# fdeguire03/InteriorPoint-GPU

Measured on AMD Instinct MI355X. Metric: Newton iters/sec, dense QP n=8192, 1/2/4/8 GPUs; achieved % fp64 roofline, higher is better.
Workload: dtype f64

## Files before the change

### interiorpoint-gpu_amd/csrc/ipm_mfma.h

```cpp
#pragma once
#include <algorithm>
#include <map>
#include <mutex>
#include <queue>
#include <tuple>
#include <type_traits>
#include <vector>

#include "ipm_common.h"

namespace ipm {

#ifdef IPM_TILE_STAMPS
__device__ unsigned long long ipm_tile_stamps[4096 * 8];
#define IPM_TSTAMP(k) do { if (threadIdx.x == 0 && blockIdx.x < 4096) ipm_tile_stamps[blockIdx.x * 8 + (k)] = __builtin_amdgcn_s_memtime(); } while (0)
#define IPM_TSTAMPR(k) do { if (threadIdx.x == 0 && blockIdx.x < 4096) ipm_tile_stamps[blockIdx.x * 8 + (k)] = __builtin_amdgcn_s_memrealtime(); } while (0)
#else
#define IPM_TSTAMP(k) do {} while (0)
#define IPM_TSTAMPR(k) do {} while (0)
#endif

struct GemmArgs {
  int64_t ni = 0, nj = 0, K = 0;
  const double* X = nullptr;
  int64_t ldx = 0;
  const double* Y = nullptr;
  int64_t ldy = 0;
  const double* w = nullptr;
  double* C = nullptr;
  int64_t ldc = 0;
  double alpha = 1.0, beta = 0.0;
  const double* P = nullptr;
  int64_t ldp = 0;
  double tP = 0.0;
  const double* dvec = nullptr;
  const int* info = nullptr;
  int tri = 0;
  int sub = 0;
  int xcd_remap = 1;
  int rowmajor = 0;
  int64_t tiles_i = 0, tiles_j = 0, nblk = 0;
  int accum = 0;
};

#define IPM_KARGS(T, name, param) \
  (void)param;                    \
  const T& name = *(const T*)__builtin_amdgcn_kernarg_segment_ptr()

__device__ __forceinline__ double ld_sc1(const double* p) {
  return __longlong_as_double((long long)__hip_atomic_load(
      reinterpret_cast<unsigned long long*>(const_cast<double*>(p)), __ATOMIC_RELAXED, __HIP_MEMORY_SCOPE_AGENT));
}
__device__ __forceinline__ void st_sc1(double* p, double v) {
  __hip_atomic_store(reinterpret_cast<unsigned long long*>(p), (unsigned long long)__double_as_longlong(v),
                     __ATOMIC_RELAXED, __HIP_MEMORY_SCOPE_AGENT);
}

static __device__ unsigned long long ipm_spin_ticks[2] = {100000000ull, 100000000ull};
__device__ __forceinline__ void spin_fail(int* info, unsigned* failw) {
  if (info) atomicCAS(info, 0, POTRF_INFO_SPIN);
  __threadfence();
  if (failw) atomicCAS(failw, 0u, 0xFFFFFFF0u);
}
template <int SLEEP, int WHICH = 0, class Done>
__device__ __forceinline__ bool spin_until(int* info, unsigned* failw, Done done) {
  if (done()) return true;
  unsigned long long t0 = 0;
  for (unsigned it = 0;; ++it) {
    __builtin_amdgcn_s_sleep(SLEEP);
    if (done()) return true;
    if ((it & 15u) != 0u) continue;
    const unsigned long long now = __builtin_amdgcn_s_memrealtime();
    if (it == 0) {
      t0 = now;
      continue;
    }
    if (failw && __hip_atomic_load(failw, __ATOMIC_RELAXED, __HIP_MEMORY_SCOPE_AGENT) != 0u) return false;
    if (now - t0 > ipm_spin_ticks[WHICH]) {
      spin_fail(info, failw);
      return false;
    }
  }
}

#ifndef IPM_STILE_XRING
#define IPM_STILE_XRING 3
#endif

template <int BM_, int WJ = 2>
struct MfCfg {
  static constexpr int BM = BM_, BK = 16, NT = 128 * WJ;
  static constexpr int LD = BM + 16;
  static constexpr int PT = BK * BM / NT;
  static constexpr int TPR = BM / PT;
  static constexpr int TWI = BM / 32;
  static constexpr int TWJ = BM / (16 * WJ);
};

template <int BM_, int WJ = 2>
struct alignas(16) MfSmem {
  alignas(16) double sX[2][MfCfg<BM_, WJ>::BK * MfCfg<BM_, WJ>::LD];
  alignas(16) double sY[2][MfCfg<BM_, WJ>::BK * MfCfg<BM_, WJ>::LD];
};

template <int BM_, bool WEIGHT, bool VEC, int WJ = 2, bool SC1OUT = false, bool SPLITADD = false, int LOOP = 0,
          int LAZYC = 0, bool CST = false>
__device__ __forceinline__ void mfma_tile(const GemmArgs& a, int64_t Lw, MfSmem<BM_, WJ>& sm, int SPLIT = 0,
                                          double* part = nullptr, unsigned* pflag = nullptr, int64_t kb = -1,
                                          int64_t ke = -1, int* sinfo = nullptr, unsigned* failw = nullptr) {
  using M = MfCfg<BM_, WJ>;
  constexpr int BM = M::BM, BK = M::BK, LD = M::LD, PT = M::PT, TPR = M::TPR, TWI = M::TWI, TWJ = M::TWJ;
  IPM_TSTAMP(0);
  IPM_TSTAMPR(6);
#ifdef IPM_TILE_STAMPS
  if (threadIdx.x == 0 && blockIdx.x < 4096)
    ipm_tile_stamps[blockIdx.x * 8 + 5] = ((unsigned long long)__builtin_amdgcn_s_getreg((31 << 11) | 20) << 32) |
                                          __builtin_amdgcn_s_getreg((31 << 11) | 4);
#endif
  auto& sX = sm.sX;
  auto& sY = sm.sY;
  int64_t bi, bj;
  {
    int64_t L = Lw;
    const int64_t q = a.nblk >> 3;
    if (a.xcd_remap && !a.rowmajor && L < (q << 3)) L = (L & 7) * q + (L >> 3);
    if (a.rowmajor) {
      bi = L / a.tiles_j;
      bj = L % a.tiles_j;
    } else if (a.tri) {
      int64_t b = (int64_t)((sqrt(8.0 * (double)L + 1.0) - 1.0) * 0.5);
      while ((b + 1) * (b + 2) / 2 <= L) ++b;
      while (b * (b + 1) / 2 > L) --b;
      bi = b;
      bj = L - b * (b + 1) / 2;
    } else {
      bi = L % a.tiles_i;
      bj = L / a.tiles_i;
    }
  }
  const int64_t I0 = bi * BM, J0 = bj * BM;
  const bool full = (I0 + BM <= a.ni) && (J0 + BM <= a.nj);
  const int tid = threadIdx.x, lane = tid & 63, wv = tid >> 6;
  const int wi = wv & 1, wj = wv >> 1;
  const int sr = tid / TPR, sc = (tid % TPR) * PT;
  const bool kpiece = SPLITADD && kb >= 0;
  const int64_t kbeg = SPLIT == 1 ? (kpiece ? kb : a.K / 2) : 0;
  const double* xp = a.X + (sr + kbeg) * a.ldx + I0 + sc;
  const double* yp = a.Y + (sr + kbeg) * a.ldy + J0 + sc;
  const int64_t xstep = BK * a.ldx, ystep = BK * a.ldy;
  int kt32 = (int)a.K;
  if (SPLIT == 1) kt32 = kpiece ? (int)(ke - kb) : kt32 - kt32 / 2;
  if (SPLIT == 2) kt32 = kt32 / 2;
  const int64_t Kt = kt32;
  const int64_t nslab = (Kt + BK - 1) / BK;
  const bool cinit = a.sub || a.accum || (a.beta == 1.0 && a.alpha == -1.0 && !a.P && !a.dvec);
  const double xsg = (cinit && !a.accum) ? -1.0 : 1.0;
  double rx[PT], ry[PT];
  auto gload = [&](int64_t s) {
    const int64_t k = s * BK + sr;
    const double* xs = xp + s * xstep;
    const double* ys = yp + s * ystep;
    if (full && (s + 1) * BK <= Kt) {
      const double wk = WEIGHT ? a.w[kbeg + k] : 1.0;
      if (VEC) {
#pragma unroll
        for (int q = 0; q < PT / 2; ++q) {
          const double2 u = reinterpret_cast<const double2*>(xs)[q];
          const double2 v = reinterpret_cast<const double2*>(ys)[q];
          rx[2 * q] = (WEIGHT ? u.x * wk : u.x) * xsg;
          rx[2 * q + 1] = (WEIGHT ? u.y * wk : u.y) * xsg;
          ry[2 * q] = v.x;
          ry[2 * q + 1] = v.y;
        }
      } else {
#pragma unroll
        for (int q = 0; q < PT; ++q) {
          rx[q] = (WEIGHT ? xs[q] * wk : xs[q]) * xsg;
          ry[q] = ys[q];
        }
      }
    } else {
      const bool kin = k < Kt;
      const double wk = (WEIGHT && kin) ? a.w[kbeg + k] : 1.0;
#pragma unroll
      for (int q = 0; q < PT; ++q) {
        const bool xi = kin && (I0 + sc + q < a.ni), yj = kin && (J0 + sc + q < a.nj);
        rx[q] = xi ? (WEIGHT ? xs[q] * wk : xs[q]) * xsg : 0.0;
        ry[q] = yj ? ys[q] : 0.0;
      }
    }
  };
  auto sstore = [&](int buf) {
#pragma unroll
    for (int q = 0; q < PT; ++q) {
      sX[buf][sr * LD + sc + q] = rx[q];
      sY[buf][sr * LD + sc + q] = ry[q];
    }
  };
  const int fr = lane & 15, fk = lane >> 4;
  dbl4 acc[TWJ][TWI];
#pragma unroll
  for (int u = 0; u < TWJ; ++u)
#pragma unroll
    for (int v = 0; v < TWI; ++v) acc[u][v] = dbl4{0.0, 0.0, 0.0, 0.0};
  static_assert(!LAZYC || ((LOOP == 1 || LOOP == 2) && !WEIGHT), "lazy C: a fast loop, no weight");
  static_assert(!CST || (LOOP == 1 && !LAZYC && BM_ == 128 && WJ == 2), "staged C: 128-tile fast loop");
  constexpr int CLD = 144;
  double* sCst = &sm.sX[0][0];
  static_assert(!CST || 4 * BK * LD >= 64 * CLD, "staging fits the slab buffers");
  if (CST && cinit && SPLIT == 0) {
#pragma unroll
    for (int h = 0; h < 2; ++h) {
#pragma unroll
      for (int q = 0; q < 16; ++q) {
        const int e = tid + 256 * q, col = e >> 6, rp = e & 63;
        const double2 v = *reinterpret_cast<const double2*>(a.C + (J0 + 64 * h + col) * a.ldc + I0 + 2 * rp);
        *reinterpret_cast<double2*>(&sCst[col * CLD + 2 * rp]) = v;
      }
      __syncthreads();
      if (wj == h) {
#pragma unroll
        for (int tj = 0; tj < TWJ; ++tj)
#pragma unroll
          for (int ti = 0; ti < TWI; ++ti)
#pragma unroll
            for (int r = 0; r < 4; ++r)
              acc[tj][ti][r] = sCst[(tj * 16 + fk + 4 * r) * CLD + wi * (BM / 2) + ti * 16 + fr];
      }
      __syncthreads();
    }
  } else if (cinit && SPLIT != 1 && !LAZYC) {
#pragma unroll
    for (int tj = 0; tj < TWJ; ++tj)
#pragma unroll
      for (int ti = 0; ti < TWI; ++ti) {
        const int64_t i = I0 + wi * (BM / 2) + ti * 16 + fr;
#pragma unroll
        for (int r = 0; r < 4; ++r) {
          const int64_t j = J0 + wj * (BM / WJ) + tj * 16 + fk + 4 * r;
          acc[tj][ti][r] = (i < a.ni && j < a.nj) ? (SC1OUT ? ld_sc1(&a.C[j * a.ldc + i]) : a.C[j * a.ldc + i]) : 0.0;
        }
      }
  }
  static_assert(LOOP == 0 || (BM_ == 128 && VEC && WJ == 2), "fast loop: 128-tiles, vector loads");
  if constexpr (LAZYC) {
    auto cload = [&](int q) {
      const int tj = q / TWI, ti = q % TWI;
      const int64_t i = I0 + wi * (BM / 2) + ti * 16 + fr;
      const int64_t j0 = J0 + wj * (BM / WJ) + tj * 16 + fk;
      dbl4 v;
#pragma unroll
      for (int r = 0; r < 4; ++r) v[r] = a.C[(j0 + 4 * r) * a.ldc + i];
      return v;
    };
    constexpr int NS = 16, R = LAZYC > 0 ? LAZYC : 1, NSL = NS * R;
    static_assert(TWJ * TWI == NS, "one accumulator block per R slabs");
    dbl4 cq[NS];
    if constexpr (LOOP == 2) {
      double fy[PT];
      auto fload = [&](int64_t s) {
        const double2* ys = reinterpret_cast<const double2*>(yp + s * ystep);
#pragma unroll
        for (int q = 0; q < PT / 2; ++q) {
          const double2 v = ys[q];
          fy[2 * q] = v.x;
          fy[2 * q + 1] = v.y;
        }
      };
      auto fstore = [&](int buf) {
#pragma unroll
        for (int q = 0; q < PT; ++q) sY[buf][sr * LD + sc + q] = fy[q];
      };
      const double* xq = a.X + (kbeg + fk) * a.ldx + I0 + wi * (BM / 2) + fr;
      constexpr int XRING = IPM_STILE_XRING, G = NSL * (BK / 4);
      double xr[XRING][TWI];
// ... 214 lines not shown
#pragma unroll
      for (int t = 0; t < TWJ; ++t) yr[kk][t] = q[t * 16];
      if (WEIGHT) wk[kk] = wq[s * BK + kk * 4];
    };
#pragma unroll
    for (int kk = 0; kk < BK / 4; ++kk) load(0, kk);
    for (int64_t s = 0; s < nslab; ++s) {
      const int64_t sn = std::min<int64_t>(s + 1, nslab - 1);
#pragma unroll
      for (int kk = 0; kk < BK / 4; ++kk) {
        double av[TWJ], bv[TWI];
#pragma unroll
        for (int t = 0; t < TWJ; ++t) av[t] = yr[kk][t];
#pragma unroll
        for (int t = 0; t < TWI; ++t) bv[t] = (WEIGHT ? xr[kk][t] * wk[kk] : xr[kk][t]) * xsg;
        load(sn, kk);
#pragma unroll
        for (int tj = 0; tj < TWJ; ++tj)
#pragma unroll
          for (int ti = 0; ti < TWI; ++ti)
            acc[tj][ti] = __builtin_amdgcn_mfma_f64_16x16x4f64(av[tj], bv[ti], acc[tj][ti], 0, 0, 0);
      }
    }
  } else {
    if (nslab > 0) {
      gload(0);
      sstore(0);
      if (nslab > 1) gload(1);
    }
    __syncthreads();
    for (int64_t s = 0; s < nslab; ++s) {
      const int buf = (int)(s & 1);
      const double* bx = sX[buf];
      const double* by = sY[buf];
  #pragma unroll
      for (int kk = 0; kk < BK / 4; ++kk) {
        double av[TWJ], bv[TWI];
  #pragma unroll
        for (int t = 0; t < TWJ; ++t) av[t] = by[(kk * 4 + fk) * LD + wj * (BM / WJ) + t * 16 + fr];
  #pragma unroll
        for (int t = 0; t < TWI; ++t) bv[t] = bx[(kk * 4 + fk) * LD + wi * (BM / 2) + t * 16 + fr];
  #pragma unroll
        for (int tj = 0; tj < TWJ; ++tj)
  #pragma unroll
          for (int ti = 0; ti < TWI; ++ti)
            acc[tj][ti] = __builtin_amdgcn_mfma_f64_16x16x4f64(av[tj], bv[ti], acc[tj][ti], 0, 0, 0);
      }
      if (s + 1 < nslab) {
        sstore(buf ^ 1);
        if (s + 2 < nslab) gload(s + 2);
      }
      __syncthreads();
    }
  }
  if (SPLIT == 2) {
    if (tid == 0)
      spin_until<2>(sinfo, failw, [&] { return __hip_atomic_load(pflag, __ATOMIC_RELAXED, __HIP_MEMORY_SCOPE_AGENT) != 0u; });
    __syncthreads();
  }
  if (CST && cinit && SPLIT == 0) {
    const bool diag = a.tri && I0 == J0;
#pragma unroll
    for (int h = 0; h < 2; ++h) {
      if (wj == h) {
#pragma unroll
        for (int tj = 0; tj < TWJ; ++tj)
#pragma unroll
          for (int ti = 0; ti < TWI; ++ti)
#pragma unroll
            for (int r = 0; r < 4; ++r)
              sCst[(tj * 16 + fk + 4 * r) * CLD + wi * (BM / 2) + ti * 16 + fr] = acc[tj][ti][r];
      }
      __syncthreads();
#pragma unroll
      for (int q = 0; q < 16; ++q) {
        const int e = tid + 256 * q, col = e >> 6, rp = e & 63;
        const double2 v = *reinterpret_cast<const double2*>(&sCst[col * CLD + 2 * rp]);
        double* cp = a.C + (J0 + 64 * h + col) * a.ldc + I0 + 2 * rp;
        const int c = 64 * h + col;
        if (!diag || 2 * rp >= c) {
          *reinterpret_cast<double2*>(cp) = v;
        } else if (2 * rp + 1 == c) {
          cp[1] = v.y;
        }
      }
      if (h == 0) __syncthreads();
    }
    return;
  }
  constexpr bool PRE = LOOP >= 2 && !LAZYC;
#pragma unroll
  for (int tj = 0; tj < TWJ; ++tj) {
    double pp[TWI][4], pc[TWI][4];
    if constexpr (PRE) {
      if (!cinit && SPLIT != 1) {
#pragma unroll
        for (int ti = 0; ti < TWI; ++ti) {
          const int64_t i = I0 + wi * (BM / 2) + ti * 16 + fr;
#pragma unroll
          for (int r = 0; r < 4; ++r) {
            const int64_t j = J0 + wj * (BM / WJ) + tj * 16 + fk + 4 * r;
            const bool ok = i < a.ni && j < a.nj && (!a.tri || i >= j);
            pp[ti][r] = (ok && a.P) ? a.P[j * a.ldp + i] : 0.0;
            pc[ti][r] = (ok && a.beta != 0.0) ? a.C[j * a.ldc + i] : 0.0;
          }
        }
      }
    }
#pragma unroll
    for (int ti = 0; ti < TWI; ++ti) {
      const int64_t i = I0 + wi * (BM / 2) + ti * 16 + fr;
#pragma unroll
      for (int r = 0; r < 4; ++r) {
        const int64_t j = J0 + wj * (BM / WJ) + tj * 16 + fk + 4 * r;
        if (SPLIT == 1) {
          st_sc1(&part[(j - J0) * BM + (i - I0)], acc[tj][ti][r]);
        } else if (i < a.ni && j < a.nj && (!a.tri || i >= j)) {
          double* cp = a.C + j * a.ldc + i;
          if (cinit) {
            double v = acc[tj][ti][r];
            if (SPLIT == 2) v += ld_sc1(&part[(j - J0) * BM + (i - I0)]);
            if (SC1OUT) st_sc1(cp, v);
            else *cp = v;
          } else {
            double av = acc[tj][ti][r];
            if (SPLITADD && SPLIT == 2) av += ld_sc1(&part[(j - J0) * BM + (i - I0)]);
            double v = a.alpha * av;
            if (a.beta != 0.0) v += a.beta * (PRE ? pc[ti][r] : *cp);
            if (a.P) v += a.tP * (PRE ? pp[ti][r] : a.P[j * a.ldp + i]);
            if (a.dvec && i == j) v += a.dvec[i];
            *cp = v;
          }
        }
      }
    }
  }
  if (SPLIT == 1) {
    asm volatile("s_waitcnt vmcnt(0)" ::: "memory");
    __syncthreads();
    if (tid == 0) __hip_atomic_store(pflag, 1u, __ATOMIC_RELAXED, __HIP_MEMORY_SCOPE_AGENT);
  }
  if (SPLIT == 2) {
    __syncthreads();
    if (tid == 0) __hip_atomic_store(pflag, 0u, __ATOMIC_RELAXED, __HIP_MEMORY_SCOPE_AGENT);
  }
#ifdef IPM_TILE_STAMPS
  IPM_TSTAMP(3);
  asm volatile("s_waitcnt vmcnt(0)" ::: "memory");
  IPM_TSTAMP(4);
  IPM_TSTAMPR(7);
#endif
}

template <int BM>
__device__ __forceinline__ bool tile_fast_ok(const GemmArgs& a, int64_t Lw) {
  int64_t L = Lw, bi, bj;
  const int64_t q = a.nblk >> 3;
  if (a.xcd_remap && !a.rowmajor && L < (q << 3)) L = (L & 7) * q + (L >> 3);
  if (a.rowmajor) {
    bi = L / a.tiles_j;
    bj = L % a.tiles_j;
  } else if (a.tri) {
    int64_t b = (int64_t)((sqrt(8.0 * (double)L + 1.0) - 1.0) * 0.5);
    while ((b + 1) * (b + 2) / 2 <= L) ++b;
    while (b * (b + 1) / 2 > L) --b;
    bi = b;
    bj = L - b * (b + 1) / 2;
  } else {
    bi = L % a.tiles_i;
    bj = L / a.tiles_i;
  }
  return (bi + 1) * BM <= a.ni && (bj + 1) * BM <= a.nj && (a.K % 16) == 0;
}

#ifndef IPM_SYRK_LOOP
#define IPM_SYRK_LOOP 2
#endif

template <int BM_, bool WEIGHT, bool VEC, int WJ = 2>
__global__ __launch_bounds__(128 * WJ, 2 / (WJ / 2)) void k_mfma_gemm(GemmArgs a) {
  if (a.info && *a.info != 0) return;
  __shared__ MfSmem<BM_, WJ> sm;
  for (int64_t Lw = blockIdx.x; Lw < a.nblk; Lw += gridDim.x) {
    if (BM_ == 128 && VEC && WJ == 2 && tile_fast_ok<BM_>(a, Lw))
      mfma_tile<BM_, WEIGHT, VEC, WJ, false, false, (BM_ == 128 && VEC && WJ == 2) ? IPM_SYRK_LOOP : 0>(a, Lw, sm);
    else
      mfma_tile<BM_, WEIGHT, VEC, WJ>(a, Lw, sm);
  }
}

template <int BM_, bool WEIGHT, bool VEC>
__global__ __launch_bounds__(256, 2) void k_mfma_gemm_split(GemmArgs a, int64_t s_full, double* sscr,
                                                            unsigned* sflag) {
  if (a.info && *a.info != 0) return;
  __shared__ MfSmem<BM_, 2> sm;
  const int64_t b = blockIdx.x;
  constexpr int FL = (BM_ == 128 && VEC) ? IPM_SYRK_LOOP : 0;
  if (b < s_full) {
    if (FL && tile_fast_ok<BM_>(a, b)) mfma_tile<BM_, WEIGHT, VEC, 2, false, true, FL>(a, b, sm);
    else mfma_tile<BM_, WEIGHT, VEC, 2, false, true>(a, b, sm);
    return;
  }
  const int64_t u = b - s_full, p = u >> 1;
  double* part = sscr + p * (int64_t)(BM_ * BM_);
  const int64_t Lw = s_full + p;
  if (FL && (a.K % 32) == 0 && tile_fast_ok<BM_>(a, Lw))
    mfma_tile<BM_, WEIGHT, VEC, 2, false, true, FL>(a, Lw, sm, (u & 1) ? 2 : 1, part, sflag + p);
  else
    mfma_tile<BM_, WEIGHT, VEC, 2, false, true>(a, Lw, sm, (u & 1) ? 2 : 1, part, sflag + p);
}

template <int BM>
__device__ __forceinline__ void tile_ij(const GemmArgs& a, int64_t Lw, int64_t& bi, int64_t& bj) {
  int64_t L = Lw;
  const int64_t q = a.nblk >> 3;
  if (a.xcd_remap && !a.rowmajor && L < (q << 3)) L = (L & 7) * q + (L >> 3);
  if (a.rowmajor) {
    bi = L / a.tiles_j;
    bj = L % a.tiles_j;
  } else if (a.tri) {
    int64_t b = (int64_t)((sqrt(8.0 * (double)L + 1.0) - 1.0) * 0.5);
    while ((b + 1) * (b + 2) / 2 <= L) ++b;
    while (b * (b + 1) / 2 > L) --b;
    bi = b;
    bj = L - b * (b + 1) / 2;
  } else {
    bi = L % a.tiles_i;
    bj = L / a.tiles_i;
  }
}

template <bool WEIGHT, bool VEC>
__global__ __launch_bounds__(256, 2) void k_mfma_gemm_streamk(GemmArgs a, int64_t s_full, int P, int64_t Kp,
                                                              int64_t npc, double* sscr, unsigned* cnt,
                                                              int pieces_last) {
  constexpr int BM = 128;
  if (a.info && *a.info != 0) return;
  __shared__ MfSmem<BM, 2> sm;
  __shared__ int slast;
  int64_t b = blockIdx.x;
  constexpr int FL = VEC ? IPM_SYRK_LOOP : 0;
  bool whole;
  if (pieces_last) {
    whole = b < s_full;
    if (!whole) b -= s_full;
  } else {
    whole = b >= npc;
  }
  if (whole) {
    const int64_t L = pieces_last ? b : b - npc;
    if (FL && tile_fast_ok<BM>(a, L)) mfma_tile<BM, WEIGHT, VEC, 2, false, true, FL>(a, L, sm);
    else mfma_tile<BM, WEIGHT, VEC, 2, false, true>(a, L, sm);
    return;
  }
  const int64_t ti = b / P, p = b - ti * P, L = s_full + ti;
  const int64_t k0 = p * Kp, k1 = std::min<int64_t>(a.K, k0 + Kp);
  double* part = sscr + b * (int64_t)(BM * BM);
  unsigned* pf = cnt + (a.nblk - s_full) + b;
  if (FL && (k0 % 16) == 0 && ((k1 - k0) % 16) == 0 && tile_fast_ok<BM>(a, L))
    mfma_tile<BM, WEIGHT, VEC, 2, false, true, FL>(a, L, sm, 1, part, pf, k0, k1);
  else
    mfma_tile<BM, WEIGHT, VEC, 2, false, true>(a, L, sm, 1, part, pf, k0, k1);
  const int tid = threadIdx.x;
  if (tid == 0)
    slast = __hip_atomic_fetch_add(&cnt[ti], 1u, __ATOMIC_RELAXED, __HIP_MEMORY_SCOPE_AGENT) == (unsigned)(P - 1);
  __syncthreads();
  if (!slast) return;
  int64_t bi, bj;
  tile_ij<BM>(a, L, bi, bj);
  const int64_t I0 = bi * BM, J0 = bj * BM;
  const bool cinit = a.sub || a.accum || (a.beta == 1.0 && a.alpha == -1.0 && !a.P && !a.dvec);
  const double* base = sscr + ti * P * (int64_t)(BM * BM);
  auto fixup = [&](auto pc) {
    constexpr int NP = decltype(pc)::value, U = NP >= 8 ? 4 : 8;
    for (int e0 = tid; e0 < BM * BM; e0 += U * 256) {
      double pv[U][NP], pp[U], cv[U];
#pragma unroll
      for (int u = 0; u < U; ++u)
#pragma unroll
        for (int q = 0; q < NP; ++q) pv[u][q] = ld_sc1(&base[q * (int64_t)(BM * BM) + e0 + 256 * u]);
      bool ok[U];
#pragma unroll
      for (int u = 0; u < U; ++u) {
        const int e = e0 + 256 * u;
        const int64_t i = I0 + (e & (BM - 1)), j = J0 + e / BM;
        ok[u] = !(i >= a.ni || j >= a.nj || (a.tri && i < j));
        pp[u] = (ok[u] && !cinit && a.P) ? a.P[j * a.ldp + i] : 0.0;
        cv[u] = (ok[u] && (cinit || a.beta != 0.0)) ? a.C[j * a.ldc + i] : 0.0;
      }
#pragma unroll
      for (int u = 0; u < U; ++u) {
        if (!ok[u]) continue;
        const int e = e0 + 256 * u;
        const int64_t i = I0 + (e & (BM - 1)), j = J0 + e / BM;
        double sum = 0.0;
#pragma unroll
        for (int q = 0; q < NP; ++q) sum += pv[u][q];
        double* cp = a.C + j * a.ldc + i;
        if (cinit) {
          *cp = cv[u] + sum;
        } else {
          double v = a.alpha * sum;
          if (a.beta != 0.0) v += a.beta * cv[u];
          if (a.P) v += a.tP * pp[u];
          if (a.dvec && i == j) v += a.dvec[i];
          *cp = v;
        }
      }
    }
  };
  if (P == 16) fixup(std::integral_constant<int, 16>{});
  else if (P == 8) fixup(std::integral_constant<int, 8>{});
  else if (P == 4) fixup(std::integral_constant<int, 4>{});
  else {
    for (int e = tid; e < BM * BM; e += 256) {
      const int il = e & (BM - 1), jl = e / BM;
      const int64_t i = I0 + il, j = J0 + jl;
      if (i >= a.ni || j >= a.nj || (a.tri && i < j)) continue;
      double pv[16];
#pragma unroll
      for (int q = 0; q < 16; ++q) pv[q] = q < P ? ld_sc1(&base[q * (int64_t)(BM * BM) + e]) : 0.0;
      double sum = 0.0;
#pragma unroll
      for (int q = 0; q < 16; ++q)
        if (q < P) sum += pv[q];
      double* cp = a.C + j * a.ldc + i;
      if (cinit) {
        *cp = *cp + sum;
      } else {
        double v = a.alpha * sum;
        if (a.beta != 0.0) v += a.beta * (*cp);
        if (a.P) v += a.tP * a.P[j * a.ldp + i];
        if (a.dvec && i == j) v += a.dvec[i];
        *cp = v;
      }
    }
  }
  IPM_TSTAMPR(7);
  if (tid == 0) __hip_atomic_store(&cnt[ti], 0u, __ATOMIC_RELAXED, __HIP_MEMORY_SCOPE_AGENT);
}

inline int streamk_mode(int64_t nt = 0, int slots = 0) {
  static const int env = [] {
    const char* e = getenv("IPM_STREAMK");
    return e ? atoi(e) : -1;
  }();
  if (env >= 0) return env;
  (void)nt;
  (void)slots;
  return 2;
}
inline int streamk_plan(int64_t nt, int slots, int64_t cap, int64_t K, int64_t& q, int64_t& Kp) {
  const int mode = streamk_mode(nt, slots);
  q = 0;
  Kp = 0;
  if (!mode || slots <= 0 || nt < slots) return 0;
  q = nt % slots;
  if (q == 0) return 0;
  const int pmax = (mode == 3 || mode == 4) ? 8 : 16;
  int P = 1;
  while (P * 2 <= pmax && q * P * 2 <= slots && q * P * 2 <= cap && K / (P * 2) >= 64) P *= 2;
  if (P < 4) return 0;
  Kp = ((K + P - 1) / P + 15) / 16 * 16;
  P = (int)((K + Kp - 1) / Kp);
  return P >= 4 ? P : 0;
}

inline int64_t gemm_split_plan(int64_t nt, int slots, int64_t cap) {
  if (nt <= 0 || slots <= 0) return 0;
  static std::mutex mu;
  static std::map<std::tuple<int64_t, int, int64_t>, int64_t> cache;
  std::lock_guard<std::mutex> lk(mu);
  const auto key = std::make_tuple(nt, slots, cap);
  auto it = cache.find(key);
  if (it != cache.end()) return it->second;
  auto mk = [&](int64_t q) {
    std::priority_queue<double, std::vector<double>, std::greater<double>> pq;
    for (int i = 0; i < slots; ++i) pq.push(0.0);
    double m = 0.0;
    auto put = [&](double d) {
      const double t = pq.top() + d;
      pq.pop();
      pq.push(t);
      m = std::max(m, t);
    };
    for (int64_t i = 0; i < nt - q; ++i) put(1.0);
    for (int64_t i = 0; i < 2 * q; ++i) put(0.55);
    return m;
  };
  double best = mk(0);
  int64_t bq = 0;
  for (int64_t q = 8; q <= std::min(nt, cap); q += 8) {
    const double m = mk(q);
    if (m < best - 0.02) {
      best = m;
      bq = q;
    }
  }
  cache[key] = bq;
  return bq;
}

template <int BM>
inline void mfma_gemm_launch_bm(hipStream_t st, GemmArgs a, bool vec) {
  const int64_t ti = (a.ni + BM - 1) / BM, tj = (a.nj + BM - 1) / BM;
  a.tiles_i = ti;
  a.nblk = a.tri ? ti * (ti + 1) / 2 : ti * tj;
  dim3 g((unsigned)a.nblk), b(256);
  if (a.w) {
    if (vec) hipLaunchKernelGGL((k_mfma_gemm<BM, true, true>), g, b, 0, st, a);
    else hipLaunchKernelGGL((k_mfma_gemm<BM, true, false>), g, b, 0, st, a);
  } else {
    if (vec) hipLaunchKernelGGL((k_mfma_gemm<BM, false, true>), g, b, 0, st, a);
    else hipLaunchKernelGGL((k_mfma_gemm<BM, false, false>), g, b, 0, st, a);
  }
}

inline void mfma_gemm_launch(hipStream_t st, GemmArgs a) {
  if (a.ni <= 0 || a.nj <= 0) return;
  const bool vec = ((a.ldx & 1) == 0) && ((a.ldy & 1) == 0) && ((((uintptr_t)a.X) & 15) == 0) &&
                   ((((uintptr_t)a.Y) & 15) == 0);
  const int64_t ti = (a.ni + 127) / 128, tj = (a.nj + 127) / 128;
  const int64_t nblk128 = a.tri ? ti * (ti + 1) / 2 : ti * tj;
  if (nblk128 >= 768) mfma_gemm_launch_bm<128>(st, a, vec);
  else mfma_gemm_launch_bm<64>(st, a, vec);
}

inline void mfma_gemm_launch_split(hipStream_t st, GemmArgs a, double* ws, int64_t cap, int slots,
                                   bool flags_zero = false) {
  if (a.ni <= 0 || a.nj <= 0) return;
  const bool vec = ((a.ldx & 1) == 0) && ((a.ldy & 1) == 0) && ((((uintptr_t)a.X) & 15) == 0) &&
                   ((((uintptr_t)a.Y) & 15) == 0);
  const int64_t ti128 = (a.ni + 127) / 128, tj128 = (a.nj + 127) / 128;
  const int64_t nblk128 = a.tri ? ti128 * (ti128 + 1) / 2 : ti128 * tj128;
  int BM = nblk128 >= 768 ? 128 : 64;
  if (BM == 64 && ws) {
    int64_t q0 = 0, K0 = 0;
    if (streamk_plan(nblk128, slots, cap, a.K, q0, K0) > 0) BM = 128;
  }
  const int64_t ti = (a.ni + BM - 1) / BM, tj = (a.nj + BM - 1) / BM;
  a.tiles_i = ti;
  a.nblk = a.tri ? ti * (ti + 1) / 2 : ti * tj;
  if (BM == 128 && ws) {
    int64_t qk = 0, Kp = 0;
    const int P = streamk_plan(a.nblk, slots, cap, a.K, qk, Kp);
    if (P > 0) {
      const int64_t s_full = a.nblk - qk, npc = qk * P;
      unsigned* cnt = reinterpret_cast<unsigned*>(ws + cap * (int64_t)(128 * 128));
      if (!flags_zero) hipMemsetAsync(cnt, 0, qk * sizeof(unsigned), st);
      dim3 g((unsigned)(npc + s_full)), blk(256);
      const int pl = (streamk_mode(a.nblk, slots) == 2 || streamk_mode(a.nblk, slots) == 4) ? 1 : 0;
      if (a.w) {
        if (vec) hipLaunchKernelGGL((k_mfma_gemm_streamk<true, true>), g, blk, 0, st, a, s_full, P, Kp, npc, ws, cnt, pl);
        else hipLaunchKernelGGL((k_mfma_gemm_streamk<true, false>), g, blk, 0, st, a, s_full, P, Kp, npc, ws, cnt, pl);
      } else {
        if (vec) hipLaunchKernelGGL((k_mfma_gemm_streamk<false, true>), g, blk, 0, st, a, s_full, P, Kp, npc, ws, cnt, pl);
        else hipLaunchKernelGGL((k_mfma_gemm_streamk<false, false>), g, blk, 0, st, a, s_full, P, Kp, npc, ws, cnt, pl);
      }
      return;
    }
  }
  const int64_t q = ws ? gemm_split_plan(a.nblk, slots, std::min<int64_t>(cap, 256)) : 0;
  if (q == 0) {
    if (BM == 128) mfma_gemm_launch_bm<128>(st, a, vec);
    else mfma_gemm_launch_bm<64>(st, a, vec);
    return;
  }
  const int64_t s_full = a.nblk - q;
  unsigned* flags = reinterpret_cast<unsigned*>(ws + cap * (int64_t)(128 * 128));
  if (!flags_zero) hipMemsetAsync(flags, 0, q * sizeof(unsigned), st);
  dim3 g((unsigned)(s_full + 2 * q)), b(256);
#define IPM_SPLIT_LAUNCH(BMv)                                                                             \
  do {                                                                                                    \
    if (a.w) {                                                                                            \
      if (vec) hipLaunchKernelGGL((k_mfma_gemm_split<BMv, true, true>), g, b, 0, st, a, s_full, ws, flags);   \
      else hipLaunchKernelGGL((k_mfma_gemm_split<BMv, true, false>), g, b, 0, st, a, s_full, ws, flags);      \
    } else {                                                                                              \
      if (vec) hipLaunchKernelGGL((k_mfma_gemm_split<BMv, false, true>), g, b, 0, st, a, s_full, ws, flags);  \
      else hipLaunchKernelGGL((k_mfma_gemm_split<BMv, false, false>), g, b, 0, st, a, s_full, ws, flags);     \
    }                                                                                                     \
  } while (0)
  if (BM == 128) IPM_SPLIT_LAUNCH(128);
  else IPM_SPLIT_LAUNCH(64);
#undef IPM_SPLIT_LAUNCH
}

}
```

Measured before the change: 124.0.

## Add diagonal-tile SYRK path computing only lower-triangle 16x16 blocks per wave

Adds a specialized kernel path for diagonal 128x128 tiles of triangular (SYRK-style) GEMMs. Each of the four waves computes exactly 9 of the 36 lower-triangle 16x16 sub-blocks, statically verified to cover the triangle, instead of the full tile. Tile ordering can now place diagonal tiles last, and a host-side load-balancing planner (diag_plan) weighs diagonal tiles at 36/64 cost when choosing between stream-K, split, or plain launches and between BM=64 and BM=128. This skips the MFMA work on upper-triangle blocks of diagonal tiles, at the cost of more template instantiations, register pressure from the unrolled per-wave schedule, and more complex scheduling heuristics.

```diff
diff --git a/interiorpoint-gpu_amd/csrc/ipm_mfma.h b/interiorpoint-gpu_amd/csrc/ipm_mfma.h
--- a/interiorpoint-gpu_amd/csrc/ipm_mfma.h
+++ b/interiorpoint-gpu_amd/csrc/ipm_mfma.h
@@ -5,6 +5,7 @@
 #include <queue>
 #include <tuple>
 #include <type_traits>
+#include <utility>
 #include <vector>
 
 #include "ipm_common.h"
@@ -42,6 +43,7 @@
   int64_t tiles_i = 0, tiles_j = 0, nblk = 0;
   int accum = 0;
 };
+constexpr int TRI_SHORT = 2, TRI_DLAST = 4;
 
 #define IPM_KARGS(T, name, param) \
   (void)param;                    \
@@ -103,8 +105,23 @@
   alignas(16) double sY[2][MfCfg<BM_, WJ>::BK * MfCfg<BM_, WJ>::LD];
 };
 
+__device__ __forceinline__ void tri_dlast_ij(const GemmArgs& a, int64_t L, int64_t& bi, int64_t& bj) {
+  const int64_t ns = a.tiles_i * (a.tiles_i - 1) / 2;
+  if (L >= ns) {
+    bi = bj = L - ns;
+    return;
+  }
+  const int64_t q = ns >> 3;
+  if (a.xcd_remap && L < (q << 3)) L = (L & 7) * q + (L >> 3);
+  int64_t b = (int64_t)((sqrt(8.0 * (double)L + 1.0) - 1.0) * 0.5);
+  while ((b + 1) * (b + 2) / 2 <= L) ++b;
+  while (b * (b + 1) / 2 > L) --b;
+  bi = b + 1;
+  bj = L - b * (b + 1) / 2;
+}
+
 template <int BM_, bool WEIGHT, bool VEC, int WJ = 2, bool SC1OUT = false, bool SPLITADD = false, int LOOP = 0,
-          int LAZYC = 0, bool CST = false>
+          int LAZYC = 0, bool CST = false, bool DLAST = false>
 __device__ __forceinline__ void mfma_tile(const GemmArgs& a, int64_t Lw, MfSmem<BM_, WJ>& sm, int SPLIT = 0,
                                           double* part = nullptr, unsigned* pflag = nullptr, int64_t kb = -1,
                                           int64_t ke = -1, int* sinfo = nullptr, unsigned* failw = nullptr) {
@@ -120,7 +137,9 @@
   auto& sX = sm.sX;
   auto& sY = sm.sY;
   int64_t bi, bj;
-  {
+  if (DLAST && (a.tri & TRI_DLAST)) {
+    tri_dlast_ij(a, Lw, bi, bj);
+  } else {
     int64_t L = Lw;
     const int64_t q = a.nblk >> 3;
     if (a.xcd_remap && !a.rowmajor && L < (q << 3)) L = (L & 7) * q + (L >> 3);
@@ -641,9 +660,13 @@
 #endif
 }
 
-template <int BM>
+template <int BM, bool DLAST = false>
 __device__ __forceinline__ bool tile_fast_ok(const GemmArgs& a, int64_t Lw) {
   int64_t L = Lw, bi, bj;
+  if (DLAST && (a.tri & TRI_DLAST)) {
+    tri_dlast_ij(a, Lw, bi, bj);
+    return (bi + 1) * BM <= a.ni && (bj + 1) * BM <= a.nj && (a.K % 16) == 0;
+  }
   const int64_t q = a.nblk >> 3;
   if (a.xcd_remap && !a.rowmajor && L < (q << 3)) L = (L & 7) * q + (L >> 3);
   if (a.rowmajor) {
@@ -662,6 +685,224 @@
   return (bi + 1) * BM <= a.ni && (bj + 1) * BM <= a.nj && (a.K % 16) == 0;
 }
 
+template <int W>
+struct DiagPart;
+template <>
+struct DiagPart<0> {
+  static constexpr int NX = 5, NY = 2;
+  static constexpr int xr[5] = {4, 5, 6, 7, 0}, yc[5] = {0, 1, 0, 0, 0};
+  static constexpr int bx[9] = {0, 0, 1, 1, 2, 2, 3, 3, 4}, by[9] = {0, 1, 0, 1, 0, 1, 0, 1, 0};
+};
+template <>
+struct DiagPart<1> {
+  static constexpr int NX = 5, NY = 3;
+  static constexpr int xr[5] = {4, 5, 6, 7, 1}, yc[5] = {2, 3, 1, 0, 0};
+  static constexpr int bx[9] = {0, 0, 1, 1, 2, 2, 3, 3, 4}, by[9] = {0, 1, 0, 1, 0, 1, 0, 1, 2};
+};
+template <>
+struct DiagPart<2> {
+  static constexpr int NX = 4, NY = 5;
+  static constexpr int xr[5] = {1, 2, 3, 4, 0}, yc[5] = {0, 1, 2, 3, 4};
+  static constexpr int bx[9] = {0, 1, 1, 1, 2, 2, 2, 2, 3}, by[9] = {0, 0, 1, 2, 0, 1, 2, 3, 4};
+};
+template <>
+struct DiagPart<3> {
+  static constexpr int NX = 3, NY = 4;
+  static constexpr int xr[5] = {5, 6, 7, 0, 0}, yc[5] = {4, 5, 6, 7, 0};
+  static constexpr int bx[9] = {0, 0, 1, 1, 1, 2, 2, 2, 2}, by[9] = {0, 1, 0, 1, 2, 0, 1, 2, 3};
+};
+template <int W>
+constexpr unsigned long long diag_part_mask() {
+  using P = DiagPart<W>;
+  unsigned long long m = 0;
+  for (int n = 0; n < 9; ++n) {
+    const int br = P::xr[P::bx[n]], bc = P::yc[P::by[n]];
+    if (P::bx[n] >= P::NX || P::by[n] >= P::NY || br < bc || ((m >> (8 * br + bc)) & 1ull)) return 0;
+    m |= 1ull << (8 * br + bc);
+  }
+  return m;
+}
+constexpr unsigned long long diag_lower_mask() {
+  unsigned long long m = 0;
+  for (int br = 0; br < 8; ++br)
+    for (int bc = 0; bc <= br; ++bc) m |= 1ull << (8 * br + bc);
+  return m;
+}
+static_assert((diag_part_mask<0>() & diag_part_mask<1>()) == 0 && (diag_part_mask<2>() & diag_part_mask<3>()) == 0 &&
+                  ((diag_part_mask<0>() | diag_part_mask<1>()) & (diag_part_mask<2>() | diag_part_mask<3>())) == 0 &&
+                  (diag_part_mask<0>() | diag_part_mask<1>() | diag_part_mask<2>() | diag_part_mask<3>()) ==
+                      diag_lower_mask(),
+              "the four waves' blocks: an exact 9 / 9 / 9 / 9 cover of the lower triangle");
+
+template <class F, int... I>
+__device__ __forceinline__ void static_for_impl(F&& f, std::integer_sequence<int, I...>) {
+  (f(std::integral_constant<int, I>{}), ...);
+}
+template <int N, class F>
+__device__ __forceinline__ void static_for(F&& f) {
+  static_for_impl(f, std::make_integer_sequence<int, N>{});
+}
+
+template <int W, bool WEIGHT>
+__device__ __forceinline__ void mfma_diag_wave(const GemmArgs& a, int64_t I0, MfSmem<128, 2>& sm) {
+  using M = MfCfg<128, 2>;
+  using P = DiagPart<W>;
+  constexpr int BK = M::BK, LD = M::LD, PT = M::PT, TPR = M::TPR, NX = P::NX, NY = P::NY, NB = 9;
+  auto& sY = sm.sY;
+  const int64_t J0 = I0;
+  const int tid = threadIdx.x, lane = tid & 63;
+  const int sr = tid / TPR, sc = (tid % TPR) * PT;
+  const int fr = lane & 15, fk = lane >> 4;
+  const double* yp = a.Y + sr * a.ldy + J0 + sc;
+  const int64_t ystep = BK * a.ldy;
+  const int64_t nslab = a.K / BK;
+  const bool cinit = a.sub || a.accum || (a.beta == 1.0 && a.alpha == -1.0 && !a.P && !a.dvec);
+  const double xsg = (cinit && !a.accum) ? -1.0 : 1.0;
+  dbl4 acc[NB];
+#pragma unroll
+  for (int n = 0; n < NB; ++n) acc[n] = dbl4{0.0, 0.0, 0.0, 0.0};
+  if (cinit) {
+    static_for<NB>([&](auto ic) {
+      constexpr int n = decltype(ic)::value, br = P::xr[P::bx[n]], bc = P::yc[P::by[n]];
+      const int64_t i = I0 + br * 16 + fr;
+#pragma unroll
+      for (int r = 0; r < 4; ++r) acc[n][r] = a.C[(J0 + bc * 16 + fk + 4 * r) * a.ldc + i];
+    });
+  }
+  double fy[PT];
+  auto fload = [&](int64_t s) {
+    const double2* ys = reinterpret_cast<const double2*>(yp + s * ystep);
+#pragma unroll
+    for (int q = 0; q < PT / 2; ++q) {
+      const double2 v = ys[q];
+      fy[2 * q] = v.x;
+      fy[2 * q + 1] = v.y;
+    }
+  };
+  auto fstore = [&](int buf) {
+#pragma unroll
+    for (int q = 0; q < PT; ++q) sY[buf][sr * LD + sc + q] = fy[q];
+  };
+  const double* xq = a.X + fk * a.ldx + I0 + fr;
+  const double* wq = WEIGHT ? a.w + fk : nullptr;
+  double xr[BK / 4][NX], wk[BK / 4];
+  auto xload = [&](int64_t s, int kk) {
+    const double* p = xq + (s * BK + kk * 4) * a.ldx;
+    static_for<NX>([&](auto tc) {
+      constexpr int t = decltype(tc)::value;
+      xr[kk][t] = p[P::xr[t] * 16];
+    });
+    if (WEIGHT) wk[kk] = wq[s * BK + kk * 4];
+  };
+  fload(0);
+  fstore(0);
+  fload(nslab > 1 ? 1 : 0);
+#pragma unroll
+  for (int kk = 0; kk < BK / 4; ++kk) xload(0, kk);
+  __syncthreads();
+  IPM_TSTAMP(1);
+  for (int64_t s = 0; s < nslab; ++s) {
+    const int buf = (int)(s & 1);
+    const double* by = sY[buf];
+    fstore(buf ^ 1);
+    fload(std::min<int64_t>(s + 2, nslab - 1));
+    const int64_t sn = std::min<int64_t>(s + 1, nslab - 1);
+    __builtin_amdgcn_sched_barrier(0);
+#pragma unroll
+    for (int kk = 0; kk < BK / 4; ++kk) {
+      double av[NY], bv[NX];
+      static_for<NY>([&](auto tc) {
+        constexpr int t = decltype(tc)::value;
+        av[t] = by[(kk * 4 + fk) * LD + P::yc[t] * 16 + fr];
+      });
+#pragma unroll
+      for (int t = 0; t < NX; ++t) bv[t] = (WEIGHT ? xr[kk][t] * wk[kk] : xr[kk][t]) * xsg;
+      xload(sn, kk);
+      static_for<NB>([&](auto ic) {
+        constexpr int n = decltype(ic)::value;
+        acc[n] = __builtin_amdgcn_mfma_f64_16x16x4f64(av[P::by[n]], bv[P::bx[n]], acc[n], 0, 0, 0);
+      });
+    }
+    __syncthreads();
+  }
+  IPM_TSTAMP(2);
+  static_for<NB / 3>([&](auto gc) {
+    constexpr int g = decltype(gc)::value;
+    double pp[3][4], pc[3][4];
+    if (!cinit) {
+      static_for<3>([&](auto uc) {
+        constexpr int u = decltype(uc)::value, n = 3 * g + u, br = P::xr[P::bx[n]], bc = P::yc[P::by[n]];
+        const int64_t i = I0 + br * 16 + fr;
+#pragma unroll
+        for (int r = 0; r < 4; ++r) {
+          const int64_t j = J0 + bc * 16 + fk + 4 * r;
+          const bool ok = br > bc || i >= j;
+          pp[u][r] = (ok && a.P) ? a.P[j * a.ldp + i] : 0.0;
+          pc[u][r] = (ok && a.beta != 0.0) ? a.C[j * a.ldc + i] : 0.0;
+        }
+      });
+    }
+    static_for<3>([&](auto uc) {
+      constexpr int u = decltype(uc)::value, n = 3 * g + u, br = P::xr[P::bx[n]], bc = P::yc[P::by[n]];
+      const int64_t i = I0 + br * 16 + fr;
+#pragma unroll
+      for (int r = 0; r < 4; ++r) {
+        const int64_t j = J0 + bc * 16 + fk + 4 * r;
+        if (br > bc || i >= j) {
+          double* cp = a.C + j * a.ldc + i;
+          if (cinit) {
+            *cp = acc[n][r];
+          } else {
+            double v = a.alpha * acc[n][r];
+            if (a.beta != 0.0) v += a.beta * pc[u][r];
+            if (a.P) v += a.tP * pp[u][r];
+            if (a.dvec && i == j) v += a.dvec[i];
+            *cp = v;
+          }
+        }
+      }
+    });
+  });
+}
+
+template <bool WEIGHT>
+__device__ __forceinline__ void mfma_tile_diag(const GemmArgs& a, int64_t I0, MfSmem<128, 2>& sm) {
+  IPM_TSTAMP(0);
+  IPM_TSTAMPR(6);
+  switch (__builtin_amdgcn_readfirstlane((int)(threadIdx.x >> 6))) {
+    case 0: mfma_diag_wave<0, WEIGHT>(a, I0, sm); break;
+    case 1: mfma_diag_wave<1, WEIGHT>(a, I0, sm); break;
+    case 2: mfma_diag_wave<2, WEIGHT>(a, I0, sm); break;
+    default: mfma_diag_wave<3, WEIGHT>(a, I0, sm); break;
+  }
+#ifdef IPM_TILE_STAMPS
+  IPM_TSTAMP(3);
+  asm volatile("s_waitcnt vmcnt(0)" ::: "memory");
+  IPM_TSTAMP(4);
+  IPM_TSTAMPR(7);
+#endif
+}
+
+template <int BM>
+__device__ __forceinline__ bool tile_diag_ok(const GemmArgs& a, int64_t Lw, int64_t& I0) {
+  if (BM != 128 || !(a.tri & TRI_SHORT)) return false;
+  int64_t bi, bj;
+  if (a.tri & TRI_DLAST) {
+    tri_dlast_ij(a, Lw, bi, bj);
+  } else {
+    int64_t L = Lw;
+    const int64_t q = a.nblk >> 3;
+    if (a.xcd_remap && L < (q << 3)) L = (L & 7) * q + (L >> 3);
+    int64_t b = (int64_t)((sqrt(8.0 * (double)L + 1.0) - 1.0) * 0.5);
+    while ((b + 1) * (b + 2) / 2 <= L) ++b;
+    while (b * (b + 1) / 2 > L) --b;
+    bi = b;
+    bj = L - b * (b + 1) / 2;
+  }
+  I0 = bi * 128;
+  return bi == bj && I0 + 128 <= a.ni && a.K >= 16 && (a.K % 16) == 0;
+}
+
 #ifndef IPM_SYRK_LOOP
 #define IPM_SYRK_LOOP 2
 #endif
@@ -678,6 +919,16 @@
   }
 }
 
+template <bool WEIGHT>
+__global__ __launch_bounds__(256, 2) void k_mfma_syrk_diag(GemmArgs a) {
+  if (a.info && *a.info != 0) return;
+  __shared__ MfSmem<128, 2> sm;
+  const int64_t Lw = blockIdx.x;
+  int64_t D0;
+  if (tile_diag_ok<128>(a, Lw, D0)) mfma_tile_diag<WEIGHT>(a, D0, sm);
+  else mfma_tile<128, WEIGHT, true, 2, false, false, IPM_SYRK_LOOP, 0, false, true>(a, Lw, sm);
+}
+
 template <int BM_, bool WEIGHT, bool VEC>
 __global__ __launch_bounds__(256, 2) void k_mfma_gemm_split(GemmArgs a, int64_t s_full, double* sscr,
                                                             unsigned* sflag) {
@@ -686,21 +937,32 @@
   const int64_t b = blockIdx.x;
   constexpr int FL = (BM_ == 128 && VEC) ? IPM_SYRK_LOOP : 0;
   if (b < s_full) {
-    if (FL && tile_fast_ok<BM_>(a, b)) mfma_tile<BM_, WEIGHT, VEC, 2, false, true, FL>(a, b, sm);
-    else mfma_tile<BM_, WEIGHT, VEC, 2, false, true>(a, b, sm);
+    if constexpr (BM_ == 128 && VEC) {
+      int64_t D0;
+      if (tile_diag_ok<BM_>(a, b, D0)) {
+        mfma_tile_diag<WEIGHT>(a, D0, sm);
+        return;
+      }
+    }
+    if (FL && tile_fast_ok<BM_, true>(a, b)) mfma_tile<BM_, WEIGHT, VEC, 2, false, true, FL, 0, false, true>(a, b, sm);
+    else mfma_tile<BM_, WEIGHT, VEC, 2, false, true, 0, 0, false, true>(a, b, sm);
     return;
   }
   const int64_t u = b - s_full, p = u >> 1;
   double* part = sscr + p * (int64_t)(BM_ * BM_);
   const int64_t Lw = s_full + p;
-  if (FL && (a.K % 32) == 0 && tile_fast_ok<BM_>(a, Lw))
-    mfma_tile<BM_, WEIGHT, VEC, 2, false, true, FL>(a, Lw, sm, (u & 1) ? 2 : 1, part, sflag + p);
+  if (FL && (a.K % 32) == 0 && tile_fast_ok<BM_, true>(a, Lw))
+    mfma_tile<BM_, WEIGHT, VEC, 2, false, true, FL, 0, false, true>(a, Lw, sm, (u & 1) ? 2 : 1, part, sflag + p);
   else
-    mfma_tile<BM_, WEIGHT, VEC, 2, false, true>(a, Lw, sm, (u & 1) ? 2 : 1, part, sflag + p);
+    mfma_tile<BM_, WEIGHT, VEC, 2, false, true, 0, 0, false, true>(a, Lw, sm, (u & 1) ? 2 : 1, part, sflag + p);
 }
 
 template <int BM>
 __device__ __forceinline__ void tile_ij(const GemmArgs& a, int64_t Lw, int64_t& bi, int64_t& bj) {
+  if (a.tri & TRI_DLAST) {
+    tri_dlast_ij(a, Lw, bi, bj);
+    return;
+  }
   int64_t L = Lw;
   const int64_t q = a.nblk >> 3;
   if (a.xcd_remap && !a.rowmajor && L < (q << 3)) L = (L & 7) * q + (L >> 3);
@@ -738,18 +1000,25 @@
   }
   if (whole) {
     const int64_t L = pieces_last ? b : b - npc;
-    if (FL && tile_fast_ok<BM>(a, L)) mfma_tile<BM, WEIGHT, VEC, 2, false, true, FL>(a, L, sm);
-    else mfma_tile<BM, WEIGHT, VEC, 2, false, true>(a, L, sm);
+    if constexpr (VEC) {
+      int64_t D0;
+      if (tile_diag_ok<BM>(a, L, D0)) {
+        mfma_tile_diag<WEIGHT>(a, D0, sm);
+        return;
+      }
+    }
+    if (FL && tile_fast_ok<BM, true>(a, L)) mfma_tile<BM, WEIGHT, VEC, 2, false, true, FL, 0, false, true>(a, L, sm);
+    else mfma_tile<BM, WEIGHT, VEC, 2, false, true, 0, 0, false, true>(a, L, sm);
     return;
   }
   const int64_t ti = b / P, p = b - ti * P, L = s_full + ti;
   const int64_t k0 = p * Kp, k1 = std::min<int64_t>(a.K, k0 + Kp);
   double* part = sscr + b * (int64_t)(BM * BM);
   unsigned* pf = cnt + (a.nblk - s_full) + b;
-  if (FL && (k0 % 16) == 0 && ((k1 - k0) % 16) == 0 && tile_fast_ok<BM>(a, L))
-    mfma_tile<BM, WEIGHT, VEC, 2, false, true, FL>(a, L, sm, 1, part, pf, k0, k1);
+  if (FL && (k0 % 16) == 0 && ((k1 - k0) % 16) == 0 && tile_fast_ok<BM, true>(a, L))
+    mfma_tile<BM, WEIGHT, VEC, 2, false, true, FL, 0, false, true>(a, L, sm, 1, part, pf, k0, k1);
   else
-    mfma_tile<BM, WEIGHT, VEC, 2, false, true>(a, L, sm, 1, part, pf, k0, k1);
+    mfma_tile<BM, WEIGHT, VEC, 2, false, true, 0, 0, false, true>(a, L, sm, 1, part, pf, k0, k1);
   const int tid = threadIdx.x;
   if (tid == 0)
     slast = __hip_atomic_fetch_add(&cnt[ti], 1u, __ATOMIC_RELAXED, __HIP_MEMORY_SCOPE_AGENT) == (unsigned)(P - 1);
@@ -829,11 +1098,15 @@
   if (tid == 0) __hip_atomic_store(&cnt[ti], 0u, __ATOMIC_RELAXED, __HIP_MEMORY_SCOPE_AGENT);
 }
 
-inline int streamk_mode(int64_t nt = 0, int slots = 0) {
+inline int streamk_env() {
   static const int env = [] {
     const char* e = getenv("IPM_STREAMK");
     return e ? atoi(e) : -1;
   }();
+  return env;
+}
+inline int streamk_mode(int64_t nt = 0, int slots = 0) {
+  const int env = streamk_env();
   if (env >= 0) return env;
   (void)nt;
   (void)slots;
@@ -890,11 +1163,91 @@
   return bq;
 }
 
+inline int diag_tile_mode() {
+  const char* e = getenv("IPM_DIAG_TILE");
+  if (!e) return 1;
+  return e[0] == '0' ? 0 : (e[0] == '2' ? 3 : 1);
+}
+inline bool grid128_forced() {
+  const char* e = getenv("IPM_GRID128");
+  return e && e[0] == '1';
+}
+
+struct DiagPlan {
+  int kind = 0, P = 0;
+  int64_t q = 0, Kp = 0;
+  double m0 = 0.0, m = 0.0;
+};
+inline DiagPlan diag_plan(int64_t T, int64_t ndc, int slots, int64_t cap, int64_t K) {
+  DiagPlan r;
+  const int64_t nt = T * (T + 1) / 2, ns = nt - T;
+  if (nt <= 0 || slots <= 0) return r;
+  static std::mutex mu;
+  static std::map<std::tuple<int64_t, int64_t, int, int64_t, int64_t>, DiagPlan> cache;
+  std::lock_guard<std::mutex> lk(mu);
+  const auto key = std::make_tuple(T, ndc, slots, cap, K);
+  auto it = cache.find(key);
+  if (it != cache.end()) return it->second;
+  auto mk = [&](int64_t qt, int64_t np, double pc) {
+    std::priority_queue<double, std::vector<double>, std::greater<double>> pq;
+    for (int i = 0; i < slots; ++i) pq.push(0.0);
+    double m = 0.0;
+    auto put = [&](double d) {
+      const double t = pq.top() + d;
+      pq.pop();
+      pq.push(t);
+      m = std::max(m, t);
+    };
+    for (int64_t i = 0; i < nt - qt; ++i) put((i >= ns && i - ns < ndc) ? 36.0 / 64.0 : 1.0);
+    for (int64_t i = 0; i < np; ++i) put(pc);
+    return m;
+  };
+  r.m0 = r.m = mk(0, 0, 0.0);
+  int64_t q = 0, Kp = 0;
+  const int P = streamk_plan(nt, slots, cap, K, q, Kp);
+  if (P > 0) {
+    const double m = mk(q, q * P, (double)Kp / (double)K + 0.10) + 0.20;
+    if (m < r.m - 0.02) {
+      r.kind = 1;
+      r.P = P;
+      r.q = q;
+      r.Kp = Kp;
+      r.m = m;
+    }
+  }
+  if (r.kind == 0) {
+    for (int64_t qh = 8; qh <= std::min(nt, std::min<int64_t>(cap, 256)); qh += 8) {
+      const double m = mk(qh, 2 * qh, 0.55);
+      if (m < r.m - 0.02) {
+        r.kind = 2;
+        r.q = qh;
+        r.m = m;
+      }
+    }
+  }
+  cache[key] = r;
+  return r;
+}
+
+inline int diag_args(const GemmArgs& a, bool vec) {
+  if (!a.tri || a.rowmajor || !vec || a.K < 16 || (a.K % 16) != 0) return 0;
+  return diag_tile_mode();
+}
+
 template <int BM>
 inline void mfma_gemm_launch_bm(hipStream_t st, GemmArgs a, bool vec) {
   const int64_t ti = (a.ni + BM - 1) / BM, tj = (a.nj + BM - 1) / BM;
   a.tiles_i = ti;
   a.nblk = a.tri ? ti * (ti + 1) / 2 : ti * tj;
+  if (a.tri & (TRI_SHORT | TRI_DLAST)) {
+    if (BM == 128 && vec && (a.tri & TRI_SHORT) && a.ni % 128 == 0) {
+      dim3 g((unsigned)a.nblk), b(256);
+      if (a.w) hipLaunchKernelGGL((k_mfma_syrk_diag<true>), g, b, 0, st, a);
+      else hipLaunchKernelGGL((k_mfma_syrk_diag<false>), g, b, 0, st, a);
+      return;
+    }
+    a.tri = 1;
+  }
   dim3 g((unsigned)a.nblk), b(256);
   if (a.w) {
     if (vec) hipLaunchKernelGGL((k_mfma_gemm<BM, true, true>), g, b, 0, st, a);
@@ -911,7 +1264,8 @@
                    ((((uintptr_t)a.Y) & 15) == 0);
   const int64_t ti = (a.ni + 127) / 128, tj = (a.nj + 127) / 128;
   const int64_t nblk128 = a.tri ? ti * (ti + 1) / 2 : ti * tj;
-  if (nblk128 >= 768) mfma_gemm_launch_bm<128>(st, a, vec);
+  if (a.tri) a.tri = 1 | (diag_args(a, vec) << 1);
+  if (nblk128 >= 768 || grid128_forced()) mfma_gemm_launch_bm<128>(st, a, vec);
   else mfma_gemm_launch_bm<64>(st, a, vec);
 }
 
@@ -922,17 +1276,32 @@
                    ((((uintptr_t)a.Y) & 15) == 0);
   const int64_t ti128 = (a.ni + 127) / 128, tj128 = (a.nj + 127) / 128;
   const int64_t nblk128 = a.tri ? ti128 * (ti128 + 1) / 2 : ti128 * tj128;
-  int BM = nblk128 >= 768 ? 128 : 64;
+  int BM = (nblk128 >= 768 || grid128_forced()) ? 128 : 64;
+  const int dg = diag_args(a, vec);
+  const bool dplan = (dg & 2) && ws && streamk_env() < 0;
+  const int64_t ndc = a.ni / 128;
   if (BM == 64 && ws) {
     int64_t q0 = 0, K0 = 0;
-    if (streamk_plan(nblk128, slots, cap, a.K, q0, K0) > 0) BM = 128;
-  }
+    if (streamk_plan(nblk128, slots, cap, a.K, q0, K0) > 0) {
+      BM = 128;
+    } else if (dplan && nblk128 >= slots && a.ni % 128 == 0) {
+      const int64_t t64 = (a.ni + 63) / 64, n64 = t64 * (t64 + 1) / 2;
+      if (diag_plan(ti128, ndc, slots, cap, a.K).m < 0.5 * (double)((n64 + slots - 1) / slots)) BM = 128;
+    }
+  }
+  if (a.tri) a.tri = 1 | ((BM == 128 ? dg : 0) << 1);
   const int64_t ti = (a.ni + BM - 1) / BM, tj = (a.nj + BM - 1) / BM;
   a.tiles_i = ti;
   a.nblk = a.tri ? ti * (ti + 1) / 2 : ti * tj;
-  if (BM == 128 && ws) {
+  DiagPlan dp;
+  if (BM == 128 && dplan) dp = diag_plan(ti, ndc, slots, cap, a.K);
+  if (BM == 128 && ws && (!dplan || dp.kind == 1)) {
     int64_t qk = 0, Kp = 0;
-    const int P = streamk_plan(a.nblk, slots, cap, a.K, qk, Kp);
+    int P = dplan ? dp.P : streamk_plan(a.nblk, slots, cap, a.K, qk, Kp);
+    if (dplan) {
+      qk = dp.q;
+      Kp = dp.Kp;
+    }
     if (P > 0) {
       const int64_t s_full = a.nblk - qk, npc = qk * P;
       unsigned* cnt = reinterpret_cast<unsigned*>(ws + cap * (int64_t)(128 * 128));
@@ -949,7 +1318,8 @@
       return;
     }
   }
-  const int64_t q = ws ? gemm_split_plan(a.nblk, slots, std::min<int64_t>(cap, 256)) : 0;
+  const int64_t q = !ws ? 0 : (BM == 128 && dplan) ? (dp.kind == 2 ? dp.q : 0)
+                                                    : gemm_split_plan(a.nblk, slots, std::min<int64_t>(cap, 256));
   if (q == 0) {
     if (BM == 128) mfma_gemm_launch_bm<128>(st, a, vec);
     else mfma_gemm_launch_bm<64>(st, a, vec);
```

New measurement: 124.1 (median of 2 runs). No clear change (+0.0%).
